# Wulizhou888/3DGS-RayTrace

Hardware: AMD Instinct MI355X
Metric: Mrays/s @1080p, 1M Gaussians; achieved HBM GB/s vs peak; 1→8 GPU scaling (higher is better)
Workload: dtype f32; 1 GPU; c3: 1000000 Gaussians SH-3, 1920x1080, 4 spp, COR; gaussians=1000000, width=1920, height=1080, spp=4, sh_degree=3, parallelism=1 GPU

## Files before the change

3dgs-raytrace_amd/csrc/gsrt_render.hip:

```cpp
#include <algorithm>
#include <cmath>
#include <cstdlib>
#include <cstring>
#include <vector>
#include <type_traits>

#include "gsrt_internal.hpp"
#include "gsrt_project.hpp"

namespace gsrt {

constexpr uint32_t kStack = 512;
constexpr uint32_t kGroup = 4;
constexpr uint32_t kRCap = 128;
constexpr uint32_t kRBuf = 2 * kRCap;
constexpr uint32_t kRStack = 256;
constexpr uint32_t kGCap = 896;
#ifndef GSRT_GROUP_SEGMENTS
#define GSRT_GROUP_SEGMENTS 2
#endif
constexpr uint32_t kGSegs = GSRT_GROUP_SEGMENTS;
constexpr uint32_t kGStride = kGSegs * kGCap;
constexpr uint32_t kMoreLanes = 16;
constexpr uint32_t kGBuf = 1024;
// ... 430 lines not shown
                else wave_sort<false>(keys, count);
                sorted_n = CAP;
                more = more || count > CAP;
                count = CAP;
                if (culled > count) culled = count;
                thresh = keys[CAP - 1];
                tdepth = __uint_as_float((uint32_t)(thresh >> 32));
            }
        }
#ifdef GSRT_DIAG
        ++dg_steps;
        dg_nodes += k;
#endif
        const bool act = lane < k;
        const uint32_t node = act ? stack[sp - k + lane] : 0u;
        __syncthreads();
        sp -= k;
        uint32_t np = 0, na = 0, nt = 0, nr = 0;
        uint32_t p0 = 0, p1 = 0;
        uint64_t a0 = 0, a1 = 0;
        if (act) {
            const BvhNode nd = nodes[node];
#pragma unroll
            for (int side = 0; side < 2; ++side) {
                const float* clo = side ? nd.r_lo : nd.l_lo;
                const float* chi = side ? nd.r_hi : nd.l_hi;
                const uint32_t ref = side ? nd.r_ref : nd.l_ref;
                if (leaf_fp && (ref & kLeafBit)) {
                    if (!(clo[0] <= fx1 && clo[1] >= fx0 && clo[2] <= fy1 && chi[0] >= fy0)) continue;
                } else if (box_outside(F, clo, chi)) {
                    continue;
                }
                if (ref & kLeafBit) {
                    uint64_t key;
                    if (keyfn(side ? nd.r_key : nd.l_key, ref & ~kLeafBit, key) && (!has_lo || key > lo)) {
                        ++nt;
                        if (key < thresh) { if (na == 0) a0 = key; else a1 = key; ++na; }
                        else nr = 1;
                    }
                } else if (!(depth_cull && depth_lo(zr, clo, chi) > tdepth)) {
                    if (np == 0) p0 = ref; else p1 = ref;
                    ++np;
                }
            }
        }
        uint64_t b1 = __ballot(np >= 1), b2 = __ballot(np >= 2);
        uint32_t off = popc_below(b1) + popc_below(b2);
        if (np >= 1) stack[sp + off] = p0;
        if (np >= 2) stack[sp + off + 1] = p1;
        sp += (uint32_t)__popcll(b1) + (uint32_t)__popcll(b2);
        b1 = __ballot(na >= 1); b2 = __ballot(na >= 2);
        off = popc_below(b1) + popc_below(b2);
        if (na >= 1) keys[count + off] = a0;
        if (na >= 2) keys[count + off + 1] = a1;
        count += (uint32_t)__popcll(b1) + (uint32_t)__popcll(b2);
        total += (uint32_t)__popcll(__ballot(nt >= 1)) + (uint32_t)__popcll(__ballot(nt >= 2));
        more = more || __ballot(nr != 0) != 0;
        __syncthreads();
    }
    if (res.restart) return res;
#ifdef GSRT_DIAG
    const unsigned long long dg1 = __builtin_amdgcn_s_memtime();
#endif
    if (cull) count = cull_footprints<REGSORT ? 4u : 1u>(keys, culled, count, rect);
    res.sorted = MERGE && sorted_n == CAP && !cull;
    if constexpr (MERGE) {
        if (res.sorted) merge_tail<BUF, CAP>(keys, count);
    }
    if (!res.sorted && !REGSORT) wave_sort<false>(keys, count);
#ifdef GSRT_DIAG
    if (lane == 0) {
        atomicAdd(K.a.counters + 12, dg1 - dg0);
        atomicAdd(K.a.counters + 13, __builtin_amdgcn_s_memtime() - dg1);
        atomicAdd(K.a.counters + 14, dg_steps);
        atomicAdd(K.a.counters + 15, dg_nodes);
    }
#endif
    res.total = total;
    res.more = more || count > CAP;
    res.count = count < CAP ? count : CAP;
    res.n = count;
    return res;
}

template <uint32_t CAP = kCap, uint32_t BUF = 2 * CAP, class KeyFn, bool REGSORT = false, bool MERGE = false>
__device__ GSRT_INLINE Collected collect_robust(const TileRect& rect, uint64_t lo, bool has_lo, uint64_t* keys,
                                           uint32_t* stack, KeyFn keyfn, uint32_t& restarts, bool cull = false,
                                           uint32_t stack_limit = 0, const FrontRegs& front = FrontRegs{},
                                           bool depth_cull = false) {
    if (!stack_limit) stack_limit = kargs().a.stack_limit;
    static_assert((BUF & (BUF - 1)) == 0 && BUF >= CAP + 128, "keys buffer: a power of two (wave_sort pads to one) with room for a step");
    Collected c;
    if constexpr (MERGE) {
        for (uint32_t width = 64u;; width = 1u) {
            c = collect<CAP, BUF, KeyFn, REGSORT, MERGE>(rect, lo, has_lo, keys, stack, stack_limit, width, keyfn, cull,
                                                         front, depth_cull);
            if (!c.restart || width == 1u) break;
            ++restarts;
            __syncthreads();
        }
    } else {
        c = collect<CAP, BUF, KeyFn, REGSORT, MERGE>(rect, lo, has_lo, keys, stack, stack_limit, 64u, keyfn, cull, front,
                                                     depth_cull);
        if (c.restart) {
            ++restarts;
            __syncthreads();
            c = collect<CAP, BUF, KeyFn, REGSORT, MERGE>(rect, lo, has_lo, keys, stack, stack_limit, 1u, keyfn, cull, front,
                                                         depth_cull);
        }
    }
    if (c.restart && lane_id() == 0) atomicOr(kargs().a.counters + kErrWord, 1ull);
    if (REGSORT && !c.restart && !c.sorted) wave_sort<true>(keys, c.n);
    return c;
}

__device__ GSRT_INLINE void add_counters(unsigned long long rays, unsigned long long cand, unsigned long long blended,
                                    unsigned long long term, unsigned long long rounds, unsigned long long restarts,
                                    unsigned long long maxc) {
    if (lane_id() != 0) return;
    unsigned long long* c = kargs().a.counters;
    atomicAdd(c + 0, rays);
    atomicAdd(c + 1, cand);
    atomicAdd(c + 2, blended);
    atomicAdd(c + 3, term);
    atomicAdd(c + 4, rounds);
    atomicAdd(c + 5, restarts);
    atomicAdd(c + 6, 1ull);
    atomicMax(c + 7, maxc);
}


struct Stage {
    SplatRec rec[kGroup];
    float sh[kGroup][3][16];
};
static_assert(sizeof(Stage) == kGroup * 256 && sizeof(Stage) % 1024 == 0, "whole wave-instructions of 16-B pieces");

enum class CorKind { plain, stats, depth, feat, grad, shgrad };
constexpr uint32_t kFeatWaves = 4;
constexpr uint32_t kGradWaves = GSRT_GRAD_WAVES;
constexpr uint32_t kShGradWaves = GSRT_SHGRAD_WAVES;
struct NoPayload {};
struct DepthPayload { float D; };
struct ChannelPayload { float F[16]; };
struct RgbGradPayload { float G[3]; };
template <CorKind K, bool SH, bool LUT>
struct CorVariant {
    static constexpr bool sh = SH, lut = LUT;
    static constexpr bool stats = K == CorKind::stats, depth = K == CorKind::depth;
    static constexpr bool feat = K == CorKind::feat, grad = K == CorKind::grad, shgrad = K == CorKind::shgrad;
    static_assert(!(feat || grad) || !SH, "feature and gradient frames evaluate no SH");
    static_assert(!shgrad || SH, "an SH gradient frame blends the SH rows");
    static constexpr uint32_t waves =
        shgrad ? kShGradWaves : grad ? kGradWaves : feat ? kFeatWaves : SH ? (LUT ? 4 : 6) : (LUT ? 5 : 6);
    static constexpr uint32_t row_pieces = feat ? 4u : 12u;
    static constexpr uint32_t stage_pieces = SH ? 16 * kGroup : (feat ? 8 * kGroup : 4 * kGroup);
    static constexpr uint32_t stage_ops = (stage_pieces + 63) / 64;
    using RayPayload = std::conditional_t<depth, DepthPayload, std::conditional_t<feat || grad, ChannelPayload,
                                          std::conditional_t<shgrad, RgbGradPayload, NoPayload>>>;
    using SumPayload = std::conditional_t<depth, DepthPayload, std::conditional_t<feat, ChannelPayload, NoPayload>>;
};

template <uint32_t N>
__device__ GSRT_INLINE void wait_vmcnt() { asm volatile("s_waitcnt vmcnt(%0)" ::"n"(N) : "memory"); }
template <class V>
__device__ GSRT_INLINE void wait_stage(uint32_t younger) {
    constexpr uint32_t P = V::stage_ops;
    if (younger >= 2) wait_vmcnt<2 * P>();
    else if (younger == 1) wait_vmcnt<P>();
    else wait_vmcnt<0>();
}

__device__ GSRT_INLINE uint32_t lds_read_settled(const uint32_t* p) {
    const uint32_t a = (uint32_t)(uintptr_t)(const __attribute__((address_space(3))) uint32_t*)p;
    uint32_t v;
    asm volatile("ds_read_b32 %0, %1\n\ts_waitcnt lgkmcnt(0)" : "=v"(v) : "v"(a) : "memory");
    return v;
}

template <class V>
__device__ GSRT_INLINE void stage_issue(const uint32_t* ids, uint32_t count, uint32_t g0, uint32_t lane, Stage* dst,
                                   const SplatRec* recs, const float* sh) {
    constexpr uint32_t kRecPieces = 4 * kGroup, kPieces = V::stage_pieces, kRowPieces = V::row_pieces;
#pragma unroll
    for (uint32_t i = 0; i < (kPieces + 63) / 64; ++i) {
        const uint32_t p = i * 64 + lane;
        const bool is_rec = p < kRecPieces;
        const uint32_t q = p - kRecPieces;
        uint32_t c = g0 + (is_rec ? p >> 2 : q / kRowPieces);
        c = c < count ? c : g0;
        if (p < kPieces) {
            const uint32_t id = lds_read_settled(ids + c);
            const char* base = is_rec ? reinterpret_cast<const char*>(recs) : reinterpret_cast<const char*>(sh);
            const uint32_t stride = is_rec ? 64u : kRowPieces * 16u, off = is_rec ? (p & 3) * 16u : (q % kRowPieces) * 16u;
            __builtin_amdgcn_global_load_lds((const void*)(base + (size_t)id * stride + off),
                                             (void*)(reinterpret_cast<char*>(dst) + i * 1024), 16, 0, 0);
        }
    }
}

__device__ GSRT_INLINE void list_issue(uint32_t lt, uint32_t lane, uint32_t* ids, uint32_t* hdr) {
    const KArgs& K = kargs();
    const uint32_t* src = K.a.lists + (size_t)lt * kCap;
    __builtin_amdgcn_global_load_lds((const void*)(src + lane), (void*)ids, 4, 0, 0);
    __builtin_amdgcn_global_load_lds((const void*)(src + 64 + lane), (void*)(ids + 64), 4, 0, 0);
    if (lane < 4)
        __builtin_amdgcn_global_load_lds((const void*)(reinterpret_cast<const uint32_t*>(K.a.list_hdr + lt) + lane),
                                         (void*)hdr, 4, 0, 0);
}

template <class V>
struct CorRay {
    ObjRay R;
    float pxs, pys;
    float bs[16];
    float T, C[3];
    typename V::RayPayload k;
    bool active;
    uint32_t cand, blended, term;
#ifdef GSRT_DIAG
    uint32_t dg_staged, dg_gpass, dg_contrib, dg_blend, dg_lanes_g, dg_lanes_blend;
#endif
};

__device__ GSRT_INLINE float sh_channel(const float (&bs)[16], const float (&s)[16]) {
    float a = s[0];
#pragma unroll
    for (int q = 1; q < 16; ++q) a = fmaf(bs[q], s[q], a);
    return a > 0.0f ? a : 0.0f;
}
struct ShFromStage {
    const Stage* stg;
    uint32_t c;
    __device__ GSRT_INLINE void operator()(const float (&bs)[16], float (&col)[3]) const {
#pragma unroll
        for (int ch = 0; ch < 3; ++ch) {
            const float4* s4 = reinterpret_cast<const float4*>(stg->sh[c][ch]);
            const float4 q0 = s4[0], q1 = s4[1], q2 = s4[2], q3 = s4[3];
            const float s[16] = {q0.x, q0.y, q0.z, q0.w, q1.x, q1.y, q1.z, q1.w,
                                 q2.x, q2.y, q2.z, q2.w, q3.x, q3.y, q3.z, q3.w};
            col[ch] = sh_channel(bs, s);
        }
    }
};
__device__ GSRT_INLINE bool lane_of(uint64_t mask) { return __builtin_amdgcn_inverse_ballot_w64(mask); }
__device__ GSRT_INLINE const float4* feat_row(const Stage* stg, uint32_t c) {
    return reinterpret_cast<const float4*>(&stg->sh[0][0][0]) + 4 * c;
}
template <int CTRL>
__device__ GSRT_INLINE float dpp_from(float v) {
    return __int_as_float(__builtin_amdgcn_mov_dpp(__float_as_int(v), CTRL, 0xF, 0xF, false));
}
__device__ GSRT_INLINE float grad_row_sums(const float (&t)[16]) {
    const bool b3 = lane_of(0xFF00FF00FF00FF00ull), b2 = lane_of(0xF0F0F0F0F0F0F0F0ull);
    const bool b1 = lane_of(0xCCCCCCCCCCCCCCCCull), b0 = lane_of(0xAAAAAAAAAAAAAAAAull);
    float a[8], b[4], c[2];
#pragma unroll
    for (int k = 0; k < 8; ++k) a[k] = (b3 ? t[8 + k] : t[k]) + dpp_from<0x140>(b3 ? t[k] : t[8 + k]);
#pragma unroll
    for (int k = 0; k < 4; ++k) b[k] = (b2 ? a[4 + k] : a[k]) + dpp_from<0x141>(b2 ? a[k] : a[4 + k]);
#pragma unroll
    for (int k = 0; k < 2; ++k) c[k] = (b1 ? b[2 + k] : b[k]) + dpp_from<0x4E>(b1 ? b[k] : b[2 + k]);
    return (b0 ? c[1] : c[0]) + dpp_from<0xB1>(b0 ? c[0] : c[1]);
}
__device__ GSRT_INLINE float grad_stage_sums(const float (&gs)[kGroup]) {
    static_assert(kGroup == 4, "one candidate per 16-lane row");
    typedef uint32_t u32x2 __attribute__((ext_vector_type(2)));
    const u32x2 p = __builtin_amdgcn_permlane32_swap(__float_as_uint(gs[0]), __float_as_uint(gs[2]), false, false);
    const u32x2 q = __builtin_amdgcn_permlane32_swap(__float_as_uint(gs[1]), __float_as_uint(gs[3]), false, false);
    const float u = __uint_as_float(p.x) + __uint_as_float(p.y);
    const float v = __uint_as_float(q.x) + __uint_as_float(q.y);
    const u32x2 r = __builtin_amdgcn_permlane16_swap(__float_as_uint(u), __float_as_uint(v), false, false);
    return __uint_as_float(r.x) + __uint_as_float(r.y);
}
struct GradDst { float* rows; uint32_t channels; };
struct GradStage {
    const uint32_t* ids;
    GradDst dst;
    float sums[kGroup] = {0.0f, 0.0f, 0.0f, 0.0f};
    uint32_t mask = 0;
};
struct ShGradDst { float* rows; };
struct ShGradStage {
    const uint32_t* ids;
    ShGradDst dst;
    float sums[3][kGroup] = {};
    uint32_t mask = 0;
};
__device__ GSRT_INLINE GradStage stage_of(const uint32_t* ids, const GradDst& dst) { return GradStage{ids, dst}; }
__device__ GSRT_INLINE ShGradStage stage_of(const uint32_t* ids, const ShGradDst& dst) { return ShGradStage{ids, dst}; }
template <class T>
__device__ GSRT_INLINE T& only(T& t) { return t; }
template <class V, class... G>
__device__ GSRT_INLINE uint64_t blend_hit(const Stage* stg, uint32_t c, float z, float alpha, uint64_t contrib,
                                          CorRay<V>& ray, G&... grad) {
    static_assert(sizeof...(G) == (V::grad || V::shgrad ? 1 : 0), "a gradient frame's stage, and only that");
    const float tn = ray.T * (1.0f - alpha);
    const uint64_t low = __ballot(tn < 1e-4f);
    const uint64_t term = contrib & low;
    const uint64_t blend = contrib & ~low;
    if (blend) {
        float col[3] = {1.0f, 1.0f, 1.0f};
        if (V::sh) ShFromStage{stg, c}(ray.bs, col);
        if constexpr (V::grad) {
            const float w = alpha * ray.T;
            const bool mine = lane_of(blend);
            float t[16];
#pragma unroll
            for (int q = 0; q < 16; ++q) t[q] = mine ? w * ray.k.F[q] : 0.0f;
            GradStage& gs = only(grad...);
            gs.sums[c] = grad_row_sums(t);
            gs.mask |= 1u << c;
        }
        if constexpr (V::shgrad) {
            const float w = alpha * ray.T;
            const bool mine = lane_of(blend);
            ShGradStage& gs = only(grad...);
#pragma unroll
            for (int ch = 0; ch < 3; ++ch) {
                const bool on = mine && col[ch] > 0.0f;
                const float wg = w * ray.k.G[ch];
                float t[16];
#pragma unroll
                for (int q = 0; q < 16; ++q) t[q] = on ? wg * ray.bs[q] : 0.0f;
                gs.sums[ch][c] = grad_row_sums(t);
            }
            gs.mask |= 1u << c;
        }
        if (lane_of(blend)) {
            const float w = alpha * ray.T;
            ray.C[0] = fmaf(col[0], w, ray.C[0]);
            if constexpr (!V::feat && !V::grad) {
                ray.C[1] = fmaf(col[1], w, ray.C[1]);
                ray.C[2] = fmaf(col[2], w, ray.C[2]);
            }
            if constexpr (V::depth) ray.k.D = fmaf(z, w, ray.k.D);
            if constexpr (V::feat) {
                const float4* frow = feat_row(stg, c);
#pragma unroll
                for (int q = 0; q < 4; ++q) {
                    const float4 f = frow[q];
                    ray.k.F[4 * q + 0] = fmaf(f.x, w, ray.k.F[4 * q + 0]);
                    ray.k.F[4 * q + 1] = fmaf(f.y, w, ray.k.F[4 * q + 1]);
                    ray.k.F[4 * q + 2] = fmaf(f.z, w, ray.k.F[4 * q + 2]);
                    ray.k.F[4 * q + 3] = fmaf(f.w, w, ray.k.F[4 * q + 3]);
                }
            }
            ray.T = tn;
            if (V::stats) ++ray.blended;
        }
    }
    if (term) {
        if (lane_of(term)) {
            ray.active = false;
            ray.pxs = __builtin_nanf("");
            if (V::stats) ++ray.term;
        }
    }
    return term;
}

template <class V, bool FULL, class... G>
__device__ GSRT_INLINE void shade_stage(const Stage* stg, uint32_t m, const float* lut_s, CorRay<V>& ray, G... grad) {
    constexpr bool LUT = V::lut;
    if constexpr (!V::stats) {
        float gv[kGroup];
        uint64_t okg[kGroup];
#pragma unroll
        for (uint32_t c = 0; c < kGroup; ++c) {
            const float4 q2 = reinterpret_cast<const float4*>(&stg->rec[c])[2];
            float4 q3 = reinterpret_cast<const float4*>(&stg->rec[c])[3];
            asm volatile("" : "+v"(q3.w));
            const float c2 = q3.x, cut = LUT ? kGMax : q3.y;
            const float dx = ray.pxs - q2.x, dy = ray.pys - q2.y;
            gv[c] = fmaf(c2 * dy, dy, fmaf(q2.w * dx, dy, (q2.z * dx) * dx));
            okg[c] = (FULL || c < m) ? __ballot(__float_as_uint(gv[c]) <= __float_as_uint(cut)) : 0;
        }
#ifdef GSRT_DIAG
        ray.dg_staged += __ballot(ray.active) ? m : 0u;
#endif
#pragma unroll
        for (uint32_t c = 0; c < kGroup; ++c) {
            if (!okg[c]) continue;
            float4 q0 = reinterpret_cast<const float4*>(&stg->rec[c])[0];
            const float4 q1 = reinterpret_cast<const float4*>(&stg->rec[c])[1];
            asm volatile("" : "+v"(q0.w));
            const float lo[3] = {q0.x, q0.y, q0.z}, hi[3] = {q1.x, q1.y, q1.z};
            const bool ordered = (int)__builtin_amdgcn_readfirstlane(__float_as_uint(q1.w)) >= 0;
            const uint64_t ok = okg[c] & (ordered ? __ballot(slab_hit_ordered(ray.R, lo, hi))
                                                  : __ballot(slab_hit_rel(ray.R, lo, hi)));
            const float gs = LUT ? (lane_of(ok) ? gv[c] : 0.0f) : gv[c];
            const float e = LUT ? linear_exp(lut_s, gs) : exp_neg_nocheck(-gs);
            const float a = __builtin_fminf(fabsf(q1.w) * e, 0.99f);
            const uint64_t contrib = ok & __ballot(a > kAlphaMin);
            const float alpha = lane_of(contrib) ? a : 0.0f;
#ifdef GSRT_DIAG
            ray.dg_gpass += 1u;
            ray.dg_lanes_g += (uint32_t)__popcll(okg[c]);
            ray.dg_contrib += __ballot(alpha > 0.0f) ? 1u : 0u;
            ray.dg_blend += __ballot(alpha > 0.0f && ray.T * (1.0f - alpha) >= 1e-4f) ? 1u : 0u;
            ray.dg_lanes_blend += (uint32_t)__popcll(__ballot(alpha > 0.0f && ray.T * (1.0f - alpha) >= 1e-4f));
#endif
            const uint64_t stopped = blend_hit<V>(stg, c, q0.w, alpha, contrib, ray, grad...);
            if (stopped) {
#pragma unroll
                for (uint32_t c1 = c + 1; c1 < kGroup; ++c1) okg[c1] &= ~stopped;
            }
        }
        if constexpr (V::grad) {
            const GradStage& go = only(grad...);
            const uint32_t gmask = go.mask;
            if (gmask) {
                const float sum = grad_stage_sums(go.sums);
                const uint32_t l = lane_here(), c = l >> 4, ch = l & 15u;
                if (((gmask >> c) & 1u) && ch < go.dst.channels) {
                    const uint32_t id = lds_read_settled(go.ids + c);
#if GSRT_GRAD_AB == 1
                    asm volatile("" ::"v"(sum), "v"(id));
#elif GSRT_GRAD_AB == 2
                    const float one = ch == 0 || c == (uint32_t)__builtin_ctz(gmask) ? 1.0f : 0.0f;
                    asm volatile("" ::"v"(sum));
                    atomicAdd(go.dst.rows + (size_t)id * 16u + ch, one);
#else
                    atomicAdd(go.dst.rows + (size_t)id * 16u + ch, sum);
#endif
                }
            }
        }
        if constexpr (V::shgrad) {
            const ShGradStage& go = only(grad...);
            const uint32_t gmask = go.mask;
            if (gmask) {
                float sum[3];
#pragma unroll
                for (int ch = 0; ch < 3; ++ch) sum[ch] = grad_stage_sums(go.sums[ch]);
                const uint32_t l = lane_here(), c = l >> 4, q = l & 15u;
                if ((gmask >> c) & 1u) {
                    const uint32_t id = lds_read_settled(go.ids + c);
                    float* row = go.dst.rows + (size_t)id * 48u + q;
#pragma unroll
                    for (int ch = 0; ch < 3; ++ch) atomicAdd(row + 16 * ch, sum[ch]);
                }
            }
        }
    } else {
        for (uint32_t c = 0; c < m; ++c) {
            const float4* r4 = reinterpret_cast<const float4*>(&stg->rec[c]);
            float4 q0 = r4[0], q1 = r4[1], q2 = r4[2], q3 = r4[3];
            asm volatile("" : "+v"(q1.w), "+v"(q2.x), "+v"(q2.y), "+v"(q2.z), "+v"(q2.w), "+v"(q3.x), "+v"(q3.z));
            float alpha = 0.0f;
            if (ray.active) {
                const float lo[3] = {q0.x, q0.y, q0.z}, hi[3] = {q1.x, q1.y, q1.z};
                if (slab_hit_rel(ray.R, lo, hi)) {
                    ++ray.cand;
                    const float dx = ray.pxs - q2.x, dy = ray.pys - q2.y;
                    const float g = fmaf(q3.x * dy, dy, fmaf(q2.w * dx, dy, (q2.z * dx) * dx));
                    if (g >= 0.0f && g <= kGMax) {
                        const float e = LUT ? linear_exp(lut_s, g) : exp_neg(-g);
                        float a = fabsf(q1.w) * e;
                        if (a > 0.99f) a = 0.99f;
                        if (a > kAlphaMin) alpha = a;
                    }
                }
            }
            blend_hit<V>(stg, c, q0.w, alpha, __ballot(alpha > 0.0f), ray);
        }
    }
}


template <class V, class... G>
__device__ GSRT_INLINE bool shade_sorted(const uint32_t* ids, uint32_t count, Stage* stA, Stage* stB, Stage* stC,
                             const float* lut_s, CorRay<V>& ray, const SplatRec* recs, const float* sh, G... gdst) {
    const uint32_t lane = lane_id();
    count = __builtin_amdgcn_readfirstlane(count);
    if (count == 0) return __ballot(ray.active) != 0;
    auto issue = [&](uint32_t g, Stage* dst) { stage_issue<V>(ids, count, g, lane, dst, recs, sh); };
    auto shade = [&](Stage* stg, uint32_t g) {
        const uint32_t m = count - g < kGroup ? count - g : kGroup;
        shade_stage<V, false>(stg, m, lut_s, ray, stage_of(ids + g, gdst)...);
    };
    auto shade_full = [&](Stage* stg, uint32_t g) {
        shade_stage<V, true>(stg, kGroup, lut_s, ray, stage_of(ids + g, gdst)...);
    };
    constexpr uint32_t kWaitTwo = 2 * V::stage_ops;
    auto wait = [count](uint32_t g) {
        wait_stage<V>((g + kGroup < count ? 1u : 0u) + (g + 2 * kGroup < count ? 1u : 0u));
    };
    issue(0, stA);
    if (kGroup < count) issue(kGroup, stB);
    bool live = true;
    uint32_t g0 = 0;
    if (!V::stats) {
        for (; g0 + 4 * kGroup < count; g0 += 3 * kGroup) {
            issue(g0 + 2 * kGroup, stC);
            wait_vmcnt<kWaitTwo>();
            shade_full(stA, g0);
            if (!__ballot(ray.active)) { live = false; break; }
            issue(g0 + 3 * kGroup, stA);
            wait_vmcnt<kWaitTwo>();
            shade_full(stB, g0 + kGroup);
            if (!__ballot(ray.active)) { live = false; break; }
            issue(g0 + 4 * kGroup, stB);
            wait_vmcnt<kWaitTwo>();
            shade_full(stC, g0 + 2 * kGroup);
            if (!__ballot(ray.active)) { live = false; break; }
        }
    }
    for (; live && g0 < count; g0 += 3 * kGroup) {
        if (g0 + 2 * kGroup < count) issue(g0 + 2 * kGroup, stC);
        wait(g0);
        shade(stA, g0);
        if (!__ballot(ray.active)) { live = false; break; }
        const uint32_t g1 = g0 + kGroup;
        if (g1 >= count) break;
        if (g1 + 2 * kGroup < count) issue(g1 + 2 * kGroup, stA);
        wait(g1);
        shade(stB, g1);
        if (!__ballot(ray.active)) { live = false; break; }
        const uint32_t g2 = g1 + kGroup;
        if (g2 >= count) break;
        if (g2 + 2 * kGroup < count) issue(g2 + 2 * kGroup, stB);
        wait(g2);
        shade(stC, g2);
        if (!__ballot(ray.active)) { live = false; break; }
    }
    asm volatile("s_waitcnt vmcnt(0)" ::: "memory");
    __syncthreads();
    return live;
}

__device__ GSRT_INLINE void frontier_one(const uint32_t g) {
    __shared__ uint32_t cur[2 * kFront], nxt[2 * kFront], fin[2 * kFront];
    const uint32_t lane = lane_id();
    const KArgs& K = kargs();
    if (g >= K.a.sgroups) return;
    uint32_t* out = K.a.frontier + (size_t)g * (kFront + 1);
    const uint32_t gx = g % K.a.sgroups_x, gy = g / K.a.sgroups_x;
    if (K.a.own.active) {
        const uint32_t span = kSG * K.a.fg;
        if ((gy + 1) * span <= K.a.row0 || gy * span >= K.a.row1) return;
    }
    const uint32_t span_x = kSG * K.a.fg * K.a.tw, span_y = kSG * K.a.fg * K.a.th;
    const Frustum F = make_frustum(K.ubo, (float)(gx * span_x) - 0.5f, (float)(gy * span_y) - 0.5f,
                                   (float)((gx + 1) * span_x) + 0.5f, (float)((gy + 1) * span_y) + 0.5f);
    const BvhNode* nodes = K.a.nodes;
    uint32_t ncur = 0, nfin = 0;
    {
        const float rlo[3] = {K.a.root_box[0], K.a.root_box[1], K.a.root_box[2]};
        const float rhi[3] = {K.a.root_box[3], K.a.root_box[4], K.a.root_box[5]};
        if (!box_outside(F, rlo, rhi)) {
            if (lane == 0) cur[0] = K.a.root_ref;
            ncur = 1;
        }
    }
    __syncthreads();
    while (ncur > 0) {
        uint32_t nn = 0, nf = 0;
        for (uint32_t base = 0; base < ncur; base += 64) {
            const uint32_t i = base + lane;
            uint32_t nc = 0, c0 = 0, c1 = 0;
// ... 321 lines not shown
    const uint64_t lo = ((uint64_t)gh.w << 32) | gh.z;
    uint32_t restarts = 0;
    const uint32_t limit = K.a.stack_limit < kStack ? K.a.stack_limit : kGStack;
    const Collected cl = collect_robust<kGCap, kGBuf, KeyCor, kGroupRegSort, true>(rect, lo, true, keys, stack,
                                                                                    KeyCor{}, restarts, true, limit,
                                                                                    front, true);
    if (cl.restart) return;
    uint64_t* gdst = K.a.glist + (size_t)g * kGStride + count;
    for (uint32_t i = lane; i < cl.count; i += 64) gdst[i] = keys[i];
    if (lane == 0) {
        const uint64_t gl = cl.count ? keys[cl.count - 1] : lo;
        K.a.ghdr[g] = make_uint4((count + cl.count) | (cl.more ? 0x80000000u : 0u), 0u, (uint32_t)gl, (uint32_t)(gl >> 32));
    }
}

__global__ __launch_bounds__(64) void k_collect_cor(const KArgs karg) {
    __shared__ uint64_t keys[2 * kCap];
    __shared__ uint32_t stack[kStack];
    (void)karg;
    const uint32_t lane = lane_id();
    uint32_t lt;
    TileRect rect;
    {
        const KArgs& K = kargs();
        const uint32_t t = blockIdx.x;
        if (t >= K.a.ntiles_local) return;
        lt = xcd_local_tile(t, K.a.ntiles_local);
        uint32_t tx, ty;
        band_tile(lt, K.a.row0, K.a.row1, K.a.tiles_x, tx, ty);
        rect = tile_rect(tx, ty, K.a.tw, K.a.th);
    }
    const KArgs& K = kargs();
    uint32_t* dst = K.a.lists + (size_t)lt * kCap;
    uint32_t restarts = 0;
    const Collected cl = collect_robust(rect, 0, false, keys, stack, KeyCor{}, restarts, K.a.cull2d != 0);
    const uint64_t last = cl.count ? keys[cl.count - 1] : 0ull;
    for (uint32_t i = lane; i < cl.count; i += 64) dst[i] = (uint32_t)keys[i];
    if (lane == 0)
        K.a.list_hdr[lt] = make_uint4(cl.count | (cl.more ? 0x80000000u : 0u), cl.total, (uint32_t)last, (uint32_t)(last >> 32));
}

struct CorTile {
    uint32_t lt;
    uint32_t x0, y0, tw, th, S, lgS, lgtw, lgth;
    struct Pixel { uint32_t in_tile, s, x, y; bool valid; };
    __device__ GSRT_INLINE Pixel pixel() const {
        uint32_t l = lane_id();
        asm volatile("" : "+v"(l));
        Pixel p;
        p.in_tile = l >> lgS;
        p.s = l & (S - 1u);
        p.x = x0 + (p.in_tile & (tw - 1u));
        p.y = y0 + (p.in_tile >> lgtw);
        p.valid = p.x < kargs().a.width && p.y < kargs().a.height;
        return p;
    }
    __device__ GSRT_INLINE TileRect rect_here() const {
        uint32_t tx = x0 >> lgtw, ty = y0 >> lgth;
        asm volatile("" : "+s"(tx), "+s"(ty));
        return tile_rect(tx, ty, tw, th);
    }
};

__device__ GSRT_INLINE float over_samples(float x, uint32_t ns) {
    const float nsf = (float)ns;
    return (ns & (ns - 1)) == 0 ? x * (1.0f / nsf) : x / nsf;
}

template <class V>
struct PixelSums {
    float rgba[4];
    typename V::SumPayload k;
    template <class Op>
    __device__ GSRT_INLINE void each(Op op) {
#pragma unroll
        for (int q = 0; q < 4; ++q) op(rgba[q]);
        if constexpr (V::depth) op(k.D);
        if constexpr (V::feat) {
#pragma unroll
            for (int q = 0; q < 16; ++q) op(k.F[q]);
        }
    }
    template <class Op>
    __device__ GSRT_INLINE void each_extra_at(size_t pix, Op op) {
        if constexpr (V::depth) op(k.D, kargs().a.depth_out + pix);
        if constexpr (V::feat) {
            const uint32_t C = kargs().a.feat_channels;
            float* of = kargs().a.feat_out + pix * C;
#pragma unroll
            for (int q = 0; q < 16; ++q)
                if ((uint32_t)q < C) op(k.F[q], of + q);
        }
    }
    template <class Op>
    __device__ GSRT_INLINE void each_at(float* colour, size_t pix, Op op) {
#pragma unroll
        for (int q = 0; q < 4; ++q) op(rgba[q], colour + q);
        each_extra_at(pix, op);
    }
    __device__ GSRT_INLINE void take(const CorRay<V>& ray) {
        constexpr bool grey = V::feat || V::grad;
        rgba[0] = ray.C[0]; rgba[1] = ray.C[grey ? 0 : 1]; rgba[2] = ray.C[grey ? 0 : 2]; rgba[3] = 1.0f - ray.T;
        if constexpr (V::depth) k.D = ray.k.D;
        if constexpr (V::feat) {
#pragma unroll
            for (int q = 0; q < 16; ++q) k.F[q] = ray.k.F[q];
        }
    }
};

template <class V>
__device__ GSRT_INLINE CorRay<V> cor_ray(const CorTile::Pixel& p, uint32_t S, uint32_t pass, uint32_t passes) {
    CorRay<V> ray;
    {
        const KArgs& K = kargs();
        const uint32_t sidx = pass * S + p.s;
        uint32_t seed = K.ubo.random_seed;
        for (uint32_t q = 0; q < sidx; ++q) { random_float(&seed); random_float(&seed); }
        const float jx = random_float(&seed);
        const float jy = random_float(&seed);
        ray.pxs = (float)p.x + jx;
        ray.pys = (float)p.y + jy;
        float o[3], d[3];
        gen_ray(K.ubo, ray.pxs, ray.pys, o, d);
        ray.R = make_obj_ray(d);
        if (V::sh) sh_basis(d, ray.bs);
    }
    ray.T = 1.0f;
    ray.C[0] = ray.C[1] = ray.C[2] = 0.0f;
    if constexpr (V::depth) ray.k.D = 0.0f;
    if constexpr (V::feat) {
#pragma unroll
        for (int q = 0; q < 16; ++q) ray.k.F[q] = 0.0f;
    }
    if constexpr (V::grad) {
        const KArgs& K = kargs();
        const uint32_t C = K.a.grad_channels, ns = S * passes;
        const float* gi = K.a.grad_in + ((size_t)p.y * K.a.width + p.x) * C;
#pragma unroll
        for (int q = 0; q < 16; ++q) ray.k.F[q] = p.valid && (uint32_t)q < C ? over_samples(gi[q], ns) : 0.0f;
    }
    if constexpr (V::shgrad) {
        const KArgs& K = kargs();
        const uint32_t ns = S * passes;
        const float* gi = K.a.grad_in + ((size_t)p.y * K.a.width + p.x) * 4;
#pragma unroll
        for (int ch = 0; ch < 3; ++ch) ray.k.G[ch] = p.valid ? over_samples(gi[ch], ns) : 0.0f;
    }
    ray.active = p.valid;
    if (!p.valid) ray.pxs = __builtin_nanf("");
    ray.cand = ray.blended = ray.term = 0;
#ifdef GSRT_DIAG
    ray.dg_staged = ray.dg_gpass = ray.dg_contrib = ray.dg_blend = ray.dg_lanes_g = ray.dg_lanes_blend = 0;
#endif
    return ray;
}

__device__ GSRT_INLINE Collected round_from_list(const CorTile& t, bool& prefetched, uint32_t* ids, const uint32_t* lhdr,
                                                 uint64_t& lo, uint32_t& gpos) {
    Collected cl{};
    if (!prefetched) list_issue(t.lt, lane_here(), ids, const_cast<uint32_t*>(lhdr));
    prefetched = false;
    __syncthreads();
    const uint4 h = make_uint4(lhdr[0], lhdr[1], lhdr[2], lhdr[3]);
    const uint32_t* src = kargs().a.lists + (size_t)t.lt * kCap;
    cl.count = h.x & 0x7fffffffu;
    cl.more = (h.x >> 31) != 0;
    for (uint32_t i = 128u + lane_here(); i < cl.count; i += 64) ids[i] = src[i];
    cl.total = cl.count;
    lo = ((uint64_t)h.w << 32) | h.z;
    gpos = h.y;
    __syncthreads();
    return cl;
}
__device__ GSRT_INLINE Collected round_from_group(const CorTile& t, uint32_t* ids, uint64_t& lo, uint32_t& gpos, bool& found) {
    Collected cl{};
    const KArgs& K = kargs();
    const uint32_t g = (t.y0 / t.th / K.a.fg) * K.a.groups_x + (t.x0 / t.tw / K.a.fg);
    const uint4 gh = K.a.ghdr[g];
    const uint32_t gcount = gh.x & 0x7fffffffu;
    found = gpos < gcount;
    if (!found) return cl;
    const uint64_t* gl = K.a.glist + (size_t)g * kGStride;
    const float4* fps = K.a.footprint;
    const TileRect rect_c = t.rect_here();
    uint32_t out = 0;
    while (gpos < gcount && out < kCap) {
        const uint32_t i = gpos + lane_here();
        bool keep = false;
        uint64_t key = 0;
        if (i < gcount) {
            key = gl[i];
            keep = fp_meets(fps, (uint32_t)key, rect_c);
        }
        const uint64_t b = __ballot(keep);
        const uint32_t rank = popc_below(b), n = (uint32_t)__popcll(b), room = kCap - out;
        if (keep && rank < room) ids[out + rank] = (uint32_t)key;
        if (n > room) {
            const uint64_t kb = __ballot(keep && rank < room);
            gpos += (uint32_t)(63 - __builtin_clzll(kb)) + 1u;
            out = kCap;
        } else {
            gpos = gpos + 64u < gcount ? gpos + 64u : gcount;
            out += n;
        }
    }
    cl.count = cl.total = out;
    cl.more = gpos < gcount || (gh.x >> 31) != 0;
    lo = gl[gpos - 1];
    __syncthreads();
    return cl;
}
template <class V>
__device__ GSRT_INLINE Collected round_from_traversal(const CorTile& t, uint64_t* keys, uint32_t* stack, uint32_t* ids,
                                                      uint64_t& lo, bool has_lo, uint32_t& restarts) {
    const uint32_t lim = kargs().a.stack_limit < kRStack ? kargs().a.stack_limit : kRStack;
    const Collected cl = collect_robust<kRCap, kRBuf>(t.rect_here(), lo, has_lo, keys, stack, KeyCorRec{}, restarts,
                                                      !V::stats && kargs().a.cull2d, lim, FrontRegs{}, !V::stats);
    lo = cl.count ? keys[cl.count - 1] : lo;
    const uint32_t ln = lane_here();
    for (uint32_t base = 0; base < cl.count; base += 64) {
        const uint32_t i = base + ln;
        const uint32_t v = i < cl.count ? (uint32_t)keys[i] : 0u;
        asm volatile("" ::: "memory");
        if (i < cl.count) ids[i] = v;
        asm volatile("" ::: "memory");
    }
    __syncthreads();
    return cl;
}

template <class V>
__global__ __launch_bounds__(64) __attribute__((amdgpu_waves_per_eu(V::waves)))
void k_render_cor(const KArgs karg) {
    union CorLds {
        struct { uint64_t keys[kRBuf]; uint32_t stack[kRStack]; } t;
        struct { uint32_t ids[kCap]; uint32_t hdr[4]; } l;
    };
    __shared__ CorLds L;
    __shared__ Stage stA, stB, stC;
    __shared__ float lut_s[V::lut ? 512 : 1];
    uint64_t* const keys = L.t.keys;
    uint32_t* const stack = L.t.stack;
    uint32_t* const ids = L.l.ids;
    uint32_t* const lhdr = L.l.hdr;
    const SplatRec* const recs = kargs().a.recs;
    const float* const shp = V::feat ? kargs().a.feat_rows : kargs().a.sh;
    (void)karg;
    const uint32_t lane = lane_id();
#ifdef GSRT_DIAG
    const unsigned long long diag_entry = __builtin_amdgcn_s_memtime();
    unsigned long long diag_setup = 0, diag_last = 0;
#endif
    if (V::lut) {
        const float* lut = kargs().a.lut;
        for (uint32_t i = lane; i < 512; i += 64) lut_s[i] = lut[i];
        __syncthreads();
    }
    GSRT_WT_START;
    const uint32_t t_tile0 = (uint32_t)__builtin_amdgcn_s_memrealtime();
    CorTile tile;
    uint32_t passes;
    {
        const KArgs& K = kargs();
        const uint32_t t = blockIdx.x;
        if (t >= K.a.ntiles_local) return;
        tile.lt = xcd_local_tile_perm(t, K.a.ntiles_local, K.a.run_order);
        uint32_t tx, ty;
        band_tile(tile.lt, K.a.row0, K.a.row1, K.a.tiles_x, tx, ty);
        tile.tw = K.a.tw; tile.th = K.a.th; tile.S = K.a.s_lanes; passes = K.a.passes;
        tile.x0 = tx * tile.tw; tile.y0 = ty * tile.th;
    }
    tile.lt = __builtin_amdgcn_readfirstlane(tile.lt);
    bool prefetched = false;
    if (kargs().a.prelisted) {
        list_issue(tile.lt, lane, ids, lhdr);
        prefetched = true;
    }
    tile.x0 = __builtin_amdgcn_readfirstlane(tile.x0);
    tile.y0 = __builtin_amdgcn_readfirstlane(tile.y0);
    tile.lgS = (uint32_t)__builtin_ctz(tile.S);
    tile.lgtw = (uint32_t)__builtin_ctz(tile.tw); tile.lgth = (uint32_t)__builtin_ctz(tile.th);
    const uint32_t S = tile.S;
    PixelSums<V> sums{};
    uint32_t st_cand = 0, st_blend = 0, st_term = 0, st_rounds = 0, restarts = 0, maxc = 0;
#ifdef GSRT_DIAG
    unsigned long long diag_collect = 0, diag_shade = 0;
#endif
    for (uint32_t pass = 0; pass < passes; ++pass) {
        CorRay<V> ray = cor_ray<V>(tile.pixel(), S, pass, passes);
        uint64_t lo = 0;
        bool has_lo = false;
        uint32_t gpos = 0;
        for (;;) {
#ifdef GSRT_DIAG
            const unsigned long long d0 = __builtin_amdgcn_s_memtime();
            if (!has_lo) diag_setup += d0 - (pass == 0 ? diag_entry : diag_last);
#endif
            Collected cl;
            bool listed = true;
            if (kargs().a.prelisted && !has_lo) {
                cl = round_from_list(tile, prefetched, ids, lhdr, lo, gpos);
            } else {
                listed = false;
                if (kargs().a.use_groups) cl = round_from_group(tile, ids, lo, gpos, listed);
            }
            if (!listed) cl = round_from_traversal<V>(tile, keys, stack, ids, lo, has_lo, restarts);
#ifdef GSRT_DIAG
            const unsigned long long d1 = __builtin_amdgcn_s_memtime();
            diag_collect += d1 - d0;
#endif
            ++st_rounds;
            if (cl.total > maxc) maxc = cl.total;
            bool live;
            if constexpr (V::grad)
                live = shade_sorted<V>(ids, cl.count, &stA, &stB, &stC, lut_s, ray, recs, shp,
                                       GradDst{kargs().a.grad_rows, kargs().a.grad_channels});
            else if constexpr (V::shgrad)
                live = shade_sorted<V>(ids, cl.count, &stA, &stB, &stC, lut_s, ray, recs, shp, ShGradDst{kargs().a.grad_rows});
            else
                live = shade_sorted<V>(ids, cl.count, &stA, &stB, &stC, lut_s, ray, recs, shp);
#ifdef GSRT_DIAG
            diag_last = __builtin_amdgcn_s_memtime();
            diag_shade += diag_last - d1;
#endif
            if (!cl.more || !live) break;
            has_lo = true;
            __syncthreads();
        }
        sums.take(ray);
        if (passes > 1) {
            const CorTile::Pixel p = tile.pixel();
            if (p.valid) {
                const KArgs& K = kargs();
                const size_t pix = (size_t)p.y * K.a.width + p.x;
                float4* o = (K.a.dump8 ? K.a.accum : reinterpret_cast<float4*>(K.a.out)) +
                            (K.a.packed ? (size_t)tile.lt * (tile.tw * tile.th) + p.in_tile : pix);
                if (pass > 0) sums.each_at(&o->x, pix, [](float& v, const float* home) { v = *home + v; });
                if (pass + 1 < passes) sums.each_at(&o->x, pix, [](float v, float* home) { *home = v; });
            }
        }
        st_cand += ray.cand; st_blend += ray.blended; st_term += ray.term;
#ifdef GSRT_DIAG
        if (!V::stats && lane == 0) {
            const uint32_t dg[6] = {ray.dg_staged, ray.dg_gpass, ray.dg_contrib, ray.dg_blend, ray.dg_lanes_g, ray.dg_lanes_blend};
            for (int q = 0; q < 6; ++q) atomicAdd(kargs().a.counters + 16 + q, (unsigned long long)dg[q]);
        }
#endif
    }
    if (S > 1) sums.each([](float& v) { v = v + dpp_from<0xB1>(v); });
    if (S > 2) sums.each([](float& v) { v = v + dpp_from<0x4E>(v); });
    for (uint32_t off = 4; off < S; off <<= 1) sums.each([off](float& v) { v = v + __shfl_xor(v, (int)off); });
    for (uint32_t off = 1; V::stats && off < S; off <<= 1) {
        st_cand += __shfl_xor(st_cand, (int)off);
        st_blend += __shfl_xor(st_blend, (int)off);
        st_term += __shfl_xor(st_term, (int)off);
    }
    const KArgs& K = kargs();
    const uint32_t ns = S * passes;
    const CorTile::Pixel p = tile.pixel();
    if (p.valid && p.s == 0) {
        sums.each([ns](float& v) { v = over_samples(v, ns); });
        const float4 v = make_float4(sums.rgba[0], sums.rgba[1], sums.rgba[2], sums.rgba[3]);
        const size_t pix = (size_t)p.y * K.a.width + p.x;
        const size_t idx = K.a.packed ? (size_t)tile.lt * (tile.tw * tile.th) + p.in_tile : pix;
        if (K.a.dump8) {
            const uint32_t code = dump8_code(v);
            reinterpret_cast<uint32_t*>(K.a.out)[idx] = code;
            if (code & kDump8Escape) {
                const uint32_t e = atomicAdd(&K.a.esc[0].x, 1u);
                if (e < K.a.esc_cap)
                    K.a.esc[1 + e] = make_uint4((uint32_t)idx, __float_as_uint(v.x), __float_as_uint(v.y), __float_as_uint(v.z));
            }
        } else {
            reinterpret_cast<float4*>(K.a.out)[idx] = v;
        }
        sums.each_extra_at(pix, [](float x, float* home) { *home = x; });
        if (V::stats && K.a.ray_stats)
            reinterpret_cast<uint4*>(K.a.ray_stats)[pix] = make_uint4(st_cand, st_blend, st_rounds, st_term);
    }
#ifdef GSRT_DIAG
    if (lane == 0) {
        atomicAdd(K.a.counters + 9, diag_collect);
        atomicAdd(K.a.counters + 10, diag_shade);
        const unsigned long long dend = __builtin_amdgcn_s_memtime();
        atomicAdd(K.a.counters + 11, dend - diag_entry);
        atomicAdd(K.a.counters + 1, diag_setup);
        atomicAdd(K.a.counters + 2, dend - diag_last);
    }
#endif
    if (K.a.tile_cost && lane == 0) K.a.tile_cost[tile.lt] = (uint32_t)__builtin_amdgcn_s_memrealtime() - t_tile0;
    if (V::stats) {
        const uint32_t lead = (p.valid && p.s == 0) ? 1u : 0u;
        add_counters(wave_sum(p.valid ? 1u : 0u) * passes, wave_sum(lead ? st_cand : 0u), wave_sum(lead ? st_blend : 0u),
                     wave_sum(lead ? st_term : 0u), st_rounds, restarts, maxc);
    }
    GSRT_WT_END(0, tile.lt);
}


template <bool STATS>
__global__ __launch_bounds__(64) void k_render_ref(const KArgs karg) {
    __shared__ uint64_t keys[2 * kCap];
    __shared__ uint32_t stack[kStack];
    __shared__ float lut_s[512];
    (void)karg;
    const uint32_t lane = lane_id();
    {
        const float* lut = kargs().a.lut;
        for (uint32_t i = lane; i < 512; i += 64) lut_s[i] = lut[i];
    }
    __syncthreads();
    uint32_t lt, x0, y0, samples, bounces;
    {
        const KArgs& K = kargs();
        const uint32_t t = blockIdx.x;
        if (t >= K.a.ntiles_local) return;
        lt = xcd_local_tile(t, K.a.ntiles_local);
        uint32_t tx, ty;
        band_tile(lt, K.a.row0, K.a.row1, K.a.tiles_x, tx, ty);
        x0 = tx * 8; y0 = ty * 8;
        samples = K.a.samples; bounces = K.a.bounces;
    }
    const uint32_t px = x0 + (lane & 7u), py = y0 + (lane >> 3);
    bool valid;
    float o[3];
    ObjRay R;
    float tri = kTMax;
    {
        const KArgs& K = kargs();
        valid = px < K.a.width && py < K.a.height;
        float d[3];
        gen_ray(K.ubo, (float)px, (float)py, o, d);
        R = make_obj_ray(d);
        if (K.a.tri_t && valid) tri = K.a.tri_t[(size_t)py * K.a.width + px];
    }
    const bool tri_hit = tri < kTMax;
    const float tcut = tri * R.norm;
    const TileRect rect{(float)x0 - 0.5f, (float)y0 - 0.5f, (float)(x0 + 7) + 0.5f, (float)(y0 + 7) + 0.5f};
    uint32_t restarts = 0, st_cand = 0, st_rounds = 0;
    const Collected first = collect_robust(rect, 0, false, keys, stack, KeyRef{}, restarts);
    const bool cached = first.total <= kCap;
    float Depth = 0.0f, Trans = 1.0f;
    float kd[8], ka[8];
#pragma unroll
    for (int j = 0; j < 8; ++j) { kd[j] = kKEmpty; ka[j] = -1.0f; }
    int gnum = 0;
    for (uint32_t s = 0; s < samples; ++s) {
        bool alive = valid;
        for (uint32_t b = 0; b <= bounces; ++b) {
            if (!__ballot(alive)) break;
            bool reported = tri_hit, gauss_rep = false;
            float closest = tri;
            if (alive) {
                ++st_rounds;
                gnum = 0;
#pragma unroll
                for (int j = 0; j < 8; ++j) kd[j] = kKEmpty;
            }
            uint64_t lo = 0;
            bool has_lo = false;
            for (;;) {
                Collected cl = first;
                if (!cached) cl = collect_robust(rect, lo, has_lo, keys, stack, KeyRef{}, restarts);
                const SplatRec* recs = kargs().a.recs;
                for (uint32_t c = 0; c < cl.count; ++c) {
                    const uint32_t gid = uni((uint32_t)keys[c]);
                    const SplatRec* __restrict__ r = recs + gid;
                    if (!alive) continue;
                    const float rlo[3] = {r->lo[0], r->lo[1], r->lo[2]};
                    const float rhi[3] = {r->hi[0], r->hi[1], r->hi[2]};
                    if (!slab_hit_rel_cut(R, rlo, rhi, tcut)) continue;
                    if (st_rounds == 1) ++st_cand;
                    const float depth = r->depth;
                    if (depth <= Depth) continue;
                    const float dx = (float)px - r->ppx, dy = (float)py - r->ppy;
                    const float g = 0.5f * (((r->a * dx) * dx + ((2.0f * r->b) * dx) * dy) + (r->c * dy) * dy);
                    if (g < 0.0f || g > kGMax) continue;
                    if (g != g) continue;
                    const float alpha = r->opacity * linear_exp(lut_s, g);
                    if (alpha > kAlphaMin) {
                        float nd = depth, na = alpha;
                        bool ins = false;
#pragma unroll
                        for (int j = 0; j < 8; ++j) {
                            if (kd[j] > nd) {
                                const float td = kd[j], ta = ka[j];
                                kd[j] = nd; ka[j] = na;
                                nd = td; na = ta;
                                ins = true;
                            }
                        }
                        if (ins) gnum += 1;
                        if (0.001f <= depth && (reported ? depth < closest : depth <= kTMax)) {
                            reported = gauss_rep = true;
                            closest = depth;
                        }
                    }
                }
// ... 764 lines not shown
```

profiles/diag_split.py:

```python
import os
import sys

ROOT = os.path.dirname(os.path.dirname(os.path.abspath(__file__)))
sys.path.insert(0, os.path.join(ROOT, "3dgs-raytrace_amd"))
import gsrt

cfg = sys.argv[1] if len(sys.argv) > 1 else "c3"
n, W, H, spp, with_sh = {"c3": (1_000_000, 1920, 1080, 4, True), "c2": (100_000, 1920, 1080, 1, False),
                          "c4": (1_000_000, 3840, 2160, 1, False), "c5": (5_000_000, 1920, 1080, 16, False)}[cfg]
ctx = gsrt.Context(0)
c, r, s, o, sh = gsrt.synth_cloud(gsrt.SYNTH_COR, n, 42, with_sh)
sc = gsrt.Scene.from_model(ctx, c, r, s, o, sh)
sc.build_bvh()
ubo = gsrt.camera_from_modelview(gsrt.lookat((0, 0, 0), (0, 0, -1)), 60.0, W, H, 1.0, spp, 16)
share = bool(os.environ.get("GSRT_DEBUG_RANK_OF"))
if share:
    ctx.comm_init_loopback()
for _ in range(3):
    (sc.render_sharded_async if share else sc.render_async)(ubo, gsrt.MODE_COR)
ctx.synchronize()
if share:
    sc.render_sharded(ubo, gsrt.MODE_COR, want_image=False)
else:
    sc.render(ubo, gsrt.MODE_COR)
cnt = ctx.debug_counters()
col, sha, tot = int(cnt[9]), int(cnt[10]), int(cnt[11])
print(f"{cfg}: wave-cycles collect(traversal+sort) {col / tot:.3f}  shade {sha / tot:.3f}  other {(tot - col - sha) / tot:.3f}"
      f"  (sum of per-wave s_memtime, {tot / 1e9:.2f} G)")
print(f"{cfg}: collect() wave-cycles traversal {int(cnt[12]) / 1e9:.3f} G, final cull+sort {int(cnt[13]) / 1e9:.3f} G; "
      f"steps {int(cnt[14])}, popped nodes {int(cnt[15])} (per tile: {int(cnt[14]) / (W * H * spp / 64):.1f} steps, {int(cnt[15]) / (W * H * spp / 64):.0f} nodes)")
print(f"{cfg}: k_group_list wave-cycles {int(cnt[6]) / 1e9:.3f} G, of which tile filter {int(cnt[7]) / 1e9:.3f} G; "
      f"groups with an overflowing list: {int(cnt[5])}; group list length max {int(cnt[4])}, sum {int(cnt[3])}")
ng = max(int(cnt[3]) and 1, 1)
print(f"{cfg}: k_group_list tile filter split: per-lane tile tests (incl. the chunk's footprint loads) "
      f"{int(cnt[22]) / 1e9:.3f} G, per-tile list output {int(cnt[23]) / 1e9:.3f} G; group list to HBM {int(cnt[24]) / 1e9:.3f} G")
print(f"{cfg}: wave-cycles from entry: tile+ray setup {int(cnt[1]) / tot:.3f}, reduction+store tail {int(cnt[2]) / tot:.3f}")
waves = W * H * spp / 64
st, gp, co, bl, lg, lb = (int(x) for x in cnt[16:22])
print(f"{cfg}: per wave: staged candidates {st / waves:.1f}, some lane passes g {gp / waves:.1f}, some lane alpha > 0 "
      f"{co / waves:.1f}, some lane blends (SH) {bl / waves:.1f}; lanes per g-survivor {lg / max(gp, 1):.1f}, "
      f"lanes per blending candidate {lb / max(bl, 1):.1f}")
```

Baseline: 6363 Mrays/s.

## Defer SH colour evaluation per stage and compact blends into per-lane passes

Result: faster. 6562 Mrays/s, median of 6 (+3.1%).

```diff
diff --git a/3dgs-raytrace_amd/csrc/gsrt_render.hip b/3dgs-raytrace_amd/csrc/gsrt_render.hip
--- a/3dgs-raytrace_amd/csrc/gsrt_render.hip
+++ b/3dgs-raytrace_amd/csrc/gsrt_render.hip
@@ -606,7 +606,8 @@
     static_assert(!(feat || grad) || !SH, "feature and gradient frames evaluate no SH");
     static_assert(!shgrad || SH, "an SH gradient frame blends the SH rows");
     static constexpr uint32_t waves =
-        shgrad ? kShGradWaves : grad ? kGradWaves : feat ? kFeatWaves : SH ? (LUT ? 4 : 6) : (LUT ? 5 : 6);
+        shgrad ? kShGradWaves : grad ? kGradWaves : feat ? kFeatWaves
+        : SH ? (LUT ? (K == CorKind::plain ? 5 : 4) : 6) : (LUT ? 5 : 6);
     static constexpr uint32_t row_pieces = feat ? 4u : 12u;
     static constexpr uint32_t stage_pieces = SH ? 16 * kGroup : (feat ? 8 * kGroup : 4 * kGroup);
     static constexpr uint32_t stage_ops = (stage_pieces + 63) / 64;
@@ -674,6 +675,7 @@
     uint32_t cand, blended, term;
 #ifdef GSRT_DIAG
     uint32_t dg_staged, dg_gpass, dg_contrib, dg_blend, dg_lanes_g, dg_lanes_blend;
+    uint32_t dg_stages, dg_stages_blend, dg_lane_max;
 #endif
 };
 
@@ -814,6 +816,92 @@
     return term;
 }
 
+template <class V>
+constexpr bool kShPerLane = V::sh && !V::stats && !V::shgrad;
+struct StageBlends {
+    uint64_t blend[kGroup] = {0, 0, 0, 0};
+    float w[kGroup] = {0.0f, 0.0f, 0.0f, 0.0f};
+};
+template <class V>
+__device__ GSRT_INLINE uint64_t weigh_hit(uint32_t c, float alpha, uint64_t contrib, CorRay<V>& ray, StageBlends& sb) {
+    const float tn = ray.T * (1.0f - alpha);
+    const uint64_t low = __ballot(tn < 1e-4f);
+    const uint64_t term = contrib & low;
+    const uint64_t blend = contrib & ~low;
+    sb.blend[c] = blend;
+    sb.w[c] = alpha * ray.T;
+    ray.T = lane_of(blend) ? tn : ray.T;
+    if (term) {
+        if (lane_of(term)) {
+            ray.active = false;
+            ray.pxs = __builtin_nanf("");
+        }
+    }
+    return term;
+}
+template <class V, uint32_t J>
+__device__ GSRT_INLINE bool blend_pass(const Stage* stg, const uint64_t (&at)[kGroup][kGroup], const float (&ws)[kGroup],
+                                       CorRay<V>& ray) {
+    uint64_t any = at[J][J];
+    if constexpr (J + 1 < kGroup) any |= at[J][J + 1];
+    if constexpr (J + 2 < kGroup) any |= at[J][J + 2];
+    if constexpr (J + 3 < kGroup) any |= at[J][J + 3];
+    if (!any) return false;
+#ifdef GSRT_DIAG
+    ray.dg_lane_max += 1u;
+#endif
+    if (lane_of(any)) {
+        uint32_t cj = J;
+        float w = ws[J];
+        if constexpr (J + 1 < kGroup) {
+            const bool here = lane_of(at[J][J + 1]);
+            cj = here ? J + 1 : cj, w = here ? ws[J + 1] : w;
+        }
+        if constexpr (J + 2 < kGroup) {
+            const bool here = lane_of(at[J][J + 2]);
+            cj = here ? J + 2 : cj, w = here ? ws[J + 2] : w;
+        }
+        if constexpr (J + 3 < kGroup) {
+            const bool here = lane_of(at[J][J + 3]);
+            cj = here ? J + 3 : cj, w = here ? ws[J + 3] : w;
+        }
+        float col[3];
+        ShFromStage{stg, cj}(ray.bs, col);
+        ray.C[0] = fmaf(col[0], w, ray.C[0]);
+        ray.C[1] = fmaf(col[1], w, ray.C[1]);
+        ray.C[2] = fmaf(col[2], w, ray.C[2]);
+        if constexpr (V::depth) ray.k.D = fmaf(stg->rec[cj].depth, w, ray.k.D);
+    }
+    return true;
+}
+template <class V>
+__device__ GSRT_INLINE void blend_stage(const Stage* stg, const StageBlends& sb, CorRay<V>& ray) {
+    static_assert(kGroup == 4, "two bit planes count a lane's earlier blends; blend_pass selects among four");
+    if (!(sb.blend[0] | sb.blend[1] | sb.blend[2] | sb.blend[3])) return;
+#ifdef GSRT_DIAG
+    ray.dg_stages_blend += 1u;
+#endif
+    uint64_t at[kGroup][kGroup];
+    uint64_t p0 = 0, p1 = 0;
+#pragma unroll
+    for (uint32_t c = 0; c < kGroup; ++c) {
+        const uint64_t b = sb.blend[c];
+        at[0][c] = b & ~p0 & ~p1;
+        at[1][c] = b & p0 & ~p1;
+        at[2][c] = b & ~p0 & p1;
+        at[3][c] = b & p0 & p1;
+        const uint64_t carry = p0 & b;
+        p0 ^= b;
+        p1 ^= carry;
+    }
+    float ws[kGroup] = {sb.w[0], sb.w[1], sb.w[2], sb.w[3]};
+    asm volatile("" : "+v"(ws[0]), "+v"(ws[1]), "+v"(ws[2]), "+v"(ws[3]));
+    if (!blend_pass<V, 0>(stg, at, ws, ray)) return;
+    if (!blend_pass<V, 1>(stg, at, ws, ray)) return;
+    if (!blend_pass<V, 2>(stg, at, ws, ray)) return;
+    blend_pass<V, 3>(stg, at, ws, ray);
+}
+
 template <class V, bool FULL, class... G>
 __device__ GSRT_INLINE void shade_stage(const Stage* stg, uint32_t m, const float* lut_s, CorRay<V>& ray, G... grad) {
     constexpr bool LUT = V::lut;
@@ -832,7 +920,9 @@
         }
 #ifdef GSRT_DIAG
         ray.dg_staged += __ballot(ray.active) ? m : 0u;
-#endif
+        ray.dg_stages += __ballot(ray.active) ? 1u : 0u;
+#endif
+        [[maybe_unused]] StageBlends sb;
 #pragma unroll
         for (uint32_t c = 0; c < kGroup; ++c) {
             if (!okg[c]) continue;
@@ -855,12 +945,15 @@
             ray.dg_blend += __ballot(alpha > 0.0f && ray.T * (1.0f - alpha) >= 1e-4f) ? 1u : 0u;
             ray.dg_lanes_blend += (uint32_t)__popcll(__ballot(alpha > 0.0f && ray.T * (1.0f - alpha) >= 1e-4f));
 #endif
-            const uint64_t stopped = blend_hit<V>(stg, c, q0.w, alpha, contrib, ray, grad...);
+            uint64_t stopped;
+            if constexpr (kShPerLane<V>) stopped = weigh_hit<V>(c, alpha, contrib, ray, sb);
+            else stopped = blend_hit<V>(stg, c, q0.w, alpha, contrib, ray, grad...);
             if (stopped) {
 #pragma unroll
                 for (uint32_t c1 = c + 1; c1 < kGroup; ++c1) okg[c1] &= ~stopped;
             }
         }
+        if constexpr (kShPerLane<V>) blend_stage<V>(stg, sb, ray);
         if constexpr (V::grad) {
             const GradStage& go = only(grad...);
             const uint32_t gmask = go.mask;
@@ -1488,6 +1581,7 @@
     ray.cand = ray.blended = ray.term = 0;
 #ifdef GSRT_DIAG
     ray.dg_staged = ray.dg_gpass = ray.dg_contrib = ray.dg_blend = ray.dg_lanes_g = ray.dg_lanes_blend = 0;
+    ray.dg_stages = ray.dg_stages_blend = ray.dg_lane_max = 0;
 #endif
     return ray;
 }
@@ -1681,6 +1775,8 @@
         if (!V::stats && lane == 0) {
             const uint32_t dg[6] = {ray.dg_staged, ray.dg_gpass, ray.dg_contrib, ray.dg_blend, ray.dg_lanes_g, ray.dg_lanes_blend};
             for (int q = 0; q < 6; ++q) atomicAdd(kargs().a.counters + 16 + q, (unsigned long long)dg[q]);
+            const uint32_t ds[3] = {ray.dg_stages, ray.dg_stages_blend, ray.dg_lane_max};
+            for (int q = 0; q < 3; ++q) atomicAdd(kargs().a.counters + 25 + q, (unsigned long long)ds[q]);
         }
 #endif
     }
diff --git a/profiles/diag_split.py b/profiles/diag_split.py
--- a/profiles/diag_split.py
+++ b/profiles/diag_split.py
@@ -40,3 +40,7 @@
 print(f"{cfg}: per wave: staged candidates {st / waves:.1f}, some lane passes g {gp / waves:.1f}, some lane alpha > 0 "
       f"{co / waves:.1f}, some lane blends (SH) {bl / waves:.1f}; lanes per g-survivor {lg / max(gp, 1):.1f}, "
       f"lanes per blending candidate {lb / max(bl, 1):.1f}")
+ns, nb, lm = (int(x) for x in cnt[25:28])
+if nb:
+    print(f"{cfg}: stages shaded {ns} ({ns / waves:.2f} per wave), with a blend {nb}; per shaded stage E {bl / ns:.3f} "
+          f"E' {lm / ns:.3f}; per stage with a blend E {bl / nb:.3f} E' {lm / nb:.3f}; E'/E {lm / max(bl, 1):.3f}")
```
